# buaacyw/GaussianEditor

Measured on AMD Instinct MI355X. Metric: train iters/sec (fwd+bwd of one 1080p view per GPU + grad all-reduce), 1M Gaussians @1080p, higher is better.
Workload: dtype f32; 1 GPU; synth-v1 1000000 Gaussians SH3 (M=16, s0=0.01), 1920x1080, ring-v1 8 views, one view per GPU (BASELINE.json configs[3] shape; configs[1] bicycle.ply is not available offline); gaussians=1000000, width=1920, height=1080, views_per_rank=1, parallelism=dp1-views, view_pipeline=False, tile_bounds=reference, fast_exp=False, grad_exchange=direct, grad_exchange_route=local, grad_rows=every row of every gradient written every iteration, num_rendered=0, visible=0, pixel_instances=0, sort_key_bits=45

## Files before the change

gaussianeditor_amd/csrc/gsr_blend.hip:

```cpp
#include <limits.h>

#include <atomic>
#include <type_traits>

#include "gsr_kernels.h"

namespace gsr {

struct PixelWave {
  int tile, px, py;
  bool inside;
};

__device__ __forceinline__ bool setup_wave(const BlendArgs& a, uint32_t tile, uint32_t quad, PixelWave& pw) {
  const int tx = (int)(tile % (uint32_t)a.gx), ty = (int)(tile / (uint32_t)a.gx);
  const int lane = lane_id();
  pw.tile = (int)tile;
  pw.px = tx * TILE + (int)(quad & 1u) * QUAD + (lane & 7);
  pw.py = ty * TILE + (int)(quad >> 1) * QUAD + (lane >> 3);
  pw.inside = pw.px < a.W && pw.py < a.H;
  return __any(pw.inside) != 0;
}

struct ItemBox {
// ... 487 lines not shown
      q[10] = walk.cur.r1.y;
      stage(slot, walk.cur);
    }
    if ((uint32_t)lane >= n && (uint32_t)lane < n4) {
      float* q = &spair[lane >> 1][lane & 1];
      q[0] = q[2] = q[4] = q[6] = q[8] = q[10] = 0.f;
    }
    __syncthreads();
    uint32_t evaluated = n;
    for (uint32_t j = 0; j < n4; j += GROUP) {
      if (__all(Ts < 0.0f)) {
        evaluated = j;
        break;
      }
      float ae[GROUP], om[GROUP], w[GROUP];
      bool hit[GROUP];
#pragma unroll
      for (int pp = 0; pp < GROUP / 2; ++pp) {
        const float* q = &spair[(j >> 1) + pp][0];
        pair_alpha<FAST>(*reinterpret_cast<const float4*>(q), *reinterpret_cast<const float4*>(q + 4),
                         *reinterpret_cast<const float4*>(q + 8), pfx2, pfy2, ae + 2 * pp, om + 2 * pp);
      }
#pragma unroll
      for (int u = 0; u < GROUP; ++u) asm volatile("" : "+v"(ae[u]), "+v"(om[u]));
#pragma unroll
      for (int u = 0; u < GROUP; ++u) {
        const float test_T = Ts * om[u];
        const bool A = !(test_T < 0.0001f);
        hit[u] = A && ae[u] > 0.0f;
        w[u] = ae[u] * Ts;
        Ts = A ? test_T : -__builtin_fabsf(Ts);
      }
      group(j, hit, w);
    }
    chunk_end(min(n, evaluated));
  }
}

template <bool PROFILE, bool AUX, int SPLIT, bool FAST, bool CKPT>
__device__ __forceinline__ void forward_item(const BlendArgs& a, uint32_t tile, uint32_t quad, const float bg0, const float bg1,
                                             const float bg2, uint32_t& prof_visited, uint64_t* prof_cyc) {
  PixelWave pw;
  ItemBox box;
  if (!setup_item<SPLIT>(a, tile, quad, pw, box)) return;
  quad &= 3u;
  const int lane = lane_id();
  const uint2 range = a.ranges[pw.tile];
  const float pfx = (float)pw.px, pfy = (float)pw.py;
  (void)box;
  bool done = !pw.inside;
  float T = 1.0f;
  uint32_t last_contributor = 0;
  uint32_t evaluated = 0;

  constexpr int FWD_PAIR = 24;
  __shared__ __attribute__((aligned(16))) float sp[(WAVE / 2) * FWD_PAIR];
  const uint64_t lt_mask = (1ull << lane) - 1ull;
  const f32x2 pfx2 = {pfx, pfx}, pfy2 = {pfy, pfy};
  f32x2 C01 = {0.f, 0.f}, C2D = {0.f, 0.f};
  f32x2 S01 = {0.f, 0.f};
  float S2 = 0.f;
  constexpr bool ckpt = CKPT && !AUX;
  const uint32_t pidx = (uint32_t)((pw.py & (TILE - 1)) * TILE + (pw.px & (TILE - 1)));
  const uint32_t ck_base = ckpt ? a.ck_table[tile] : CK_NONE;
  uint32_t ck_next = (ckpt && ck_base != CK_NONE) ? (uint32_t)a.ck_pos.chunk[1] : 0xffffffffu, ck_k = 1u;
  auto stage = [&](uint32_t slot, float hA, float nB, float hC, float op, float x, float y, float z, float r, float g,
                   float b, float pos) {
    float* q = sp + (slot >> 1) * FWD_PAIR + (slot & 1u);
    q[0] = hA;
    q[2] = nB;
    q[4] = hC;
    q[6] = op;
    q[8] = x;
    q[10] = y;
    q[20] = pos;
    *reinterpret_cast<float4*>(sp + (slot >> 1) * FWD_PAIR + 12 + 4 * (slot & 1u)) = make_float4(r, g, b, z);
  };
  if (range.y > range.x) {
    ChunkWalker<true, AUX> walk(a, range.x, range.y - range.x);
    for (; walk.valid(); walk.advance()) {
      const uint64_t live_m = __ballot(!done);
      if (live_m == 0) break;
      if (ckpt && walk.chunk == ck_next) {
        if (ck_k < (uint32_t)a.ck_slots) {
          if (pw.inside) a.ck_pool[((size_t)ck_base * (uint32_t)a.ck_slots + ck_k) * (TILE * TILE) + pidx] = make_float4(T, S01.x, S01.y, S2);
          S01 = f32x2{0.f, 0.f};
          S2 = 0.f;
          if (lane == 0) atomicAdd(&a.ck_work[(size_t)tile * (uint32_t)a.ck_slots + ck_k], evaluated);
        }
        ck_k++;
        ck_next = ck_k < (uint32_t)a.ck_slots ? (uint32_t)a.ck_pos.chunk[ck_k] : 0xffffffffu;
      }
      uint64_t tc0 = 0;
      if (PROFILE) {
        tc0 = __builtin_amdgcn_s_memtime();
        prof_cyc[2]++;
      }
      const bool keep = chunk_cull(live_m, pfx - (float)(lane & 7), pfy - (float)(lane >> 3), (uint32_t)lane < walk.chunk_size(), walk.cur);
      const uint64_t m = __ballot(keep);
      if (PROFILE) prof_cyc[3] += __builtin_amdgcn_s_memtime() - tc0;
      if (m == 0) continue;
      const uint32_t cnt = (uint32_t)__popcll(m);
      const uint32_t cnt4 = (cnt + GROUP - 1) & ~(uint32_t)(GROUP - 1);
      __syncthreads();
      const float csum = (walk.cur.r2.x + walk.cur.r2.y) + (walk.cur.r2.z + walk.cur.r1.z);
      const bool bad_value = keep && !(csum - csum == 0.0f);
      if (keep)
        stage((uint32_t)__popcll(m & lt_mask), -0.5f * walk.cur.r0.x, -walk.cur.r0.y, -0.5f * walk.cur.r0.z, walk.cur.r0.w,
              walk.cur.r1.x, walk.cur.r1.y, walk.cur.r1.z, walk.cur.r2.x, walk.cur.r2.y, walk.cur.r2.z,
              __uint_as_float(walk.lane_pos() + 1u));
      if ((uint32_t)lane >= cnt && (uint32_t)lane < cnt4)
        stage((uint32_t)lane, 0.f, 0.f, 0.f, 0.f, 0.f, 0.f, 0.f, 0.f, 0.f, 0.f, 0.f);
      __syncthreads();
      uint64_t tc1 = 0;
      if (PROFILE) {
        tc1 = __builtin_amdgcn_s_memtime();
        prof_cyc[0] += tc1 - tc0;
      }
      if (!__any(bad_value)) {
        float Ts = done ? -T : T;
        for (uint32_t j = 0; j < cnt4; j += GROUP) {
          if (__all(Ts < 0.0f)) break;
          evaluated += GROUP;
          if (PROFILE) prof_visited += GROUP;
          float ae[GROUP], om[GROUP], posf[GROUP];
          f32x2 rg[GROUP], bz[GROUP];
#pragma unroll
          for (int pp = 0; pp < GROUP / 2; ++pp) {
            const float* q = sp + ((j >> 1) + pp) * FWD_PAIR;
            const float4 q0 = *reinterpret_cast<const float4*>(q), q1 = *reinterpret_cast<const float4*>(q + 4),
                         q2 = *reinterpret_cast<const float4*>(q + 8), c0 = *reinterpret_cast<const float4*>(q + 12),
                         c1 = *reinterpret_cast<const float4*>(q + 16);
            const float2 ps = *reinterpret_cast<const float2*>(q + 20);
            pair_alpha<FAST>(q0, q1, q2, pfx2, pfy2, ae + 2 * pp, om + 2 * pp);
            rg[2 * pp] = f32x2{c0.x, c0.y};
            bz[2 * pp] = f32x2{c0.z, c0.w};
            rg[2 * pp + 1] = f32x2{c1.x, c1.y};
            bz[2 * pp + 1] = f32x2{c1.z, c1.w};
            posf[2 * pp] = ps.x;
            posf[2 * pp + 1] = ps.y;
          }
#pragma unroll
          for (int u = 0; u < GROUP; ++u) asm volatile("" : "+v"(ae[u]), "+v"(om[u]));
#pragma unroll
          for (int u = 0; u < GROUP; ++u) {
            const float test_T = Ts * om[u];
            const bool A = !(test_T < 0.0001f);
            const float w = ae[u] * Ts;
            const float wz = A ? w : 0.0f;
            const f32x2 w2 = {wz, wz};
            C01 = __builtin_elementwise_fma(rg[u], w2, C01);
            C2D = __builtin_elementwise_fma(bz[u], w2, C2D);
            if (ckpt) {
              S01 = __builtin_elementwise_fma(rg[u], w2, S01);
              S2 = __builtin_fmaf(bz[u].x, wz, S2);
            }
            Ts = A ? test_T : -__builtin_fabsf(Ts);
            last_contributor = (wz > 0.0f) ? __float_as_uint(posf[u]) : last_contributor;
          }
        }
        done = Ts < 0.0f;
        T = __builtin_fabsf(Ts);
      } else {
        for (uint32_t j = 0; j < cnt4; j += GROUP) {
          if (__all(done)) break;
          evaluated += GROUP;
          if (PROFILE) prof_visited += GROUP;
          float al[GROUP], om[GROUP], posf[GROUP];
          bool ok[GROUP];
          f32x2 rg[GROUP], bz[GROUP];
  #pragma unroll
          for (int pp = 0; pp < GROUP / 2; ++pp) {
            const float* q = sp + ((j >> 1) + pp) * FWD_PAIR;
            const float4 q0 = *reinterpret_cast<const float4*>(q), q1 = *reinterpret_cast<const float4*>(q + 4),
                         q2 = *reinterpret_cast<const float4*>(q + 8), c0 = *reinterpret_cast<const float4*>(q + 12),
                         c1 = *reinterpret_cast<const float4*>(q + 16);
            const float2 ps = *reinterpret_cast<const float2*>(q + 20);
            const f32x2 hA = {q0.x, q0.y}, nB = {q0.z, q0.w}, hC = {q1.x, q1.y}, op = {q1.z, q1.w};
            const f32x2 dx = f32x2{q2.x, q2.y} - pfx2, dy = f32x2{q2.z, q2.w} - pfy2;
            const f32x2 a_ = (hA * dx) * dx;
            const f32x2 s_ = __builtin_elementwise_fma(hC * dy, dy, a_);
            const f32x2 power = __builtin_elementwise_fma(nB * dx, dy, s_);
            const f32x2 e = blend_exp2<FAST>(power);
            const f32x2 ao = op * e;
            const f32x2 a2 = {fminf(0.99f, ao.x), fminf(0.99f, ao.y)};
            const f32x2 o2 = f32x2{1.0f, 1.0f} - a2;
            al[2 * pp] = a2.x;
            al[2 * pp + 1] = a2.y;
            om[2 * pp] = o2.x;
            om[2 * pp + 1] = o2.y;
            ok[2 * pp] = !(power.x > 0.0f) && !(a2.x < 1.0f / 255.0f);
            ok[2 * pp + 1] = !(power.y > 0.0f) && !(a2.y < 1.0f / 255.0f);
            rg[2 * pp] = f32x2{c0.x, c0.y};
            bz[2 * pp] = f32x2{c0.z, c0.w};
            rg[2 * pp + 1] = f32x2{c1.x, c1.y};
            bz[2 * pp + 1] = f32x2{c1.z, c1.w};
            posf[2 * pp] = ps.x;
            posf[2 * pp + 1] = ps.y;
          }
  #pragma unroll
          for (int u = 0; u < GROUP; ++u) asm volatile("" : "+v"(al[u]), "+v"(om[u]));
  #pragma unroll
          for (int u = 0; u < GROUP; ++u) {
            const bool hit = ok[u] && !done;
            const float test_T = T * om[u];
            const bool term = hit && (test_T < 0.0001f);
            done = done || term;
            if (hit && !term) {
              const float w = al[u] * T;
              const f32x2 w2 = {w, w};
              C01 = __builtin_elementwise_fma(rg[u], w2, C01);
              C2D = __builtin_elementwise_fma(bz[u], w2, C2D);
              if (ckpt) {
                S01 = __builtin_elementwise_fma(rg[u], w2, S01);
                S2 = __builtin_fmaf(bz[u].x, w, S2);
              }
              T = test_T;
              last_contributor = __float_as_uint(posf[u]);
            }
          }
        }
      }
      if (PROFILE) prof_cyc[1] += __builtin_amdgcn_s_memtime() - tc1;
    }
  }
  const float C0 = C01.x, C1 = C01.y, C2 = C2D.x, D = C2D.y;
  const uint32_t deep = (a.work_est != nullptr || ckpt) ? wave_max_u32_dpp(last_contributor) : 0u;
  if (ckpt) {
    if (deep > a.ck_pos.pos(1u) && lane == 0) atomicMax(&a.tile_maxc[tile], deep);
    if (ck_k > 1u && pw.inside)
      a.ck_pool[((size_t)ck_base * (uint32_t)a.ck_slots + (ck_k < (uint32_t)a.ck_slots ? ck_k : 0u)) * (TILE * TILE) + pidx] = make_float4(T, S01.x, S01.y, S2);
  }
  if (a.work_est != nullptr && lane == 0) {
    if (SPLIT == 1) {
      a.work_est[4u * tile + quad] = evaluated;
      a.work_maxc[4u * tile + quad] = deep;
    } else {
      atomicMax(&a.work_est[4u * tile + quad], evaluated);
      atomicMax(&a.work_maxc[4u * tile + quad], deep);
    }
  }
  if (pw.inside) {
    const size_t pix = (size_t)pw.py * a.W + pw.px, HW = (size_t)a.H * a.W;
    if (a.final_T != nullptr) {
      a.final_T[pix] = T;
      a.n_contrib[pix] = last_contributor;
    }
    a.out_color[pix] = __builtin_fmaf(T, bg0, C0);
    a.out_color[HW + pix] = __builtin_fmaf(T, bg1, C1);
    a.out_color[2 * HW + pix] = __builtin_fmaf(T, bg2, C2);
    if (a.out_depth != nullptr) a.out_depth[pix] = D;
  }
}

template <bool PROFILE, bool AUX, int SPLIT, bool FAST, bool CKPT>
__global__ void __launch_bounds__(WAVE) __attribute__((amdgpu_waves_per_eu(4, 4))) blend_forward_kernel(const BlendArgs a) {
  uint64_t t_start = 0;
  uint32_t prof_visited = 0, prof_items = 0;
  uint64_t prof_cyc[4] = {0, 0, 0, 0};
  if (PROFILE) t_start = __builtin_amdgcn_s_memtime();
  const float bg0 = wave_uniform(a.bg[0]), bg1 = wave_uniform(a.bg[1]), bg2 = wave_uniform(a.bg[2]);
  run_work_queue<SPLIT>(a, true, [&](uint32_t tile, uint32_t quad, bool empty) __attribute__((always_inline)) {
    if (PROFILE) prof_items++;
    if (!empty) {
      forward_item<PROFILE, AUX, SPLIT, FAST, CKPT>(a, tile, quad, bg0, bg1, bg2, prof_visited, prof_cyc);
    } else {
      for_each_pixel_of_tile(a, tile, [&](size_t pix, size_t HW) __attribute__((always_inline)) {
        if (a.final_T != nullptr) {
          a.final_T[pix] = 1.0f;
          a.n_contrib[pix] = 0u;
        }
        a.out_color[pix] = __builtin_fmaf(1.0f, bg0, 0.f);
        a.out_color[HW + pix] = __builtin_fmaf(1.0f, bg1, 0.f);
        a.out_color[2 * HW + pix] = __builtin_fmaf(1.0f, bg2, 0.f);
        if (a.out_depth != nullptr) a.out_depth[pix] = 0.f;
      });
    }
  });
  if (PROFILE) {
    const uint64_t t_end = __builtin_amdgcn_s_memtime();
    if (lane_id() == 0) {
      uint64_t* rec = a.profile + (size_t)blockIdx.x * 8;
      rec[4] = prof_cyc[0];
      rec[5] = prof_cyc[1];
      rec[6] = prof_cyc[2];
      rec[7] = prof_cyc[3];
      rec[0] = t_start;
      rec[1] = t_end;
      rec[2] = ((uint64_t)xcc_id() << 32) | (uint64_t)__builtin_amdgcn_s_getreg((32 - 1) << 11 | 0 << 6 | 4);
      rec[3] = ((uint64_t)prof_items << 32) | (uint64_t)prof_visited;
    }
  }
}

__device__ __forceinline__ void wave_lds_sync() {
  __builtin_amdgcn_fence(__ATOMIC_ACQ_REL, "wavefront");
  __builtin_amdgcn_wave_barrier();
}

constexpr int BWD_WAVES = 4;
constexpr int ACC_LDS_ROW = 9;
template <bool DEPTH, bool ABS = false> constexpr int bwd_moments() { return (DEPTH ? 10 : 9) + (ABS ? 2 : 0); }
template <bool DEPTH, bool ABS = false> constexpr int bwd_lds_row() { return ABS ? (DEPTH ? 13 : 11) : DEPTH ? 11 : ACC_LDS_ROW; }
constexpr uint32_t BWD_ITEM_HALF = 0x80000000u;
constexpr uint32_t BWD_ITEM_PART = 0x40000000u;
constexpr uint32_t BWD_ITEM_SEG = 0x10000000u;
static_assert(BWD_ITEM_SEG == BWD_ITEM_SEG_BIT, "gsr_kernels.h states the bit gsr_debug_blend_backward_items counts");
constexpr int BWD_SEG_SHIFT = 20, BWD_NSEG_SHIFT = 24;
static_assert(CK_MAX <= 16, "a stride index must fit the item code's 4 bits");
constexpr uint32_t BWD_ITEM_TILE = 0x000fffffu;
static_assert(BWD_ITEM_TILE + 1u == (uint32_t)GSR_MAX_TILES, "include/gsr.h states the backward's tile limit");

__device__ __forceinline__ uint4 load_backward_item(const BlendArgs& a, uint32_t index) {
  const uint32_t code = scalar_load(a.bwd_order, index);
  const uint32_t ctile = code & BWD_ITEM_TILE;
  const uint2 crange = scalar_load(a.ranges, ctile);
  const uint4 cmax = scalar_load(reinterpret_cast<const uint4*>(a.work_maxc), ctile);
  const uint32_t r01 = max(cmax.x, cmax.y), r23 = max(cmax.z, cmax.w);
  return make_uint4(code, crange.x, (code & BWD_ITEM_HALF) ? ((code & BWD_ITEM_PART) ? r23 : r01) : max(r01, r23), crange.y - crange.x);
}
__device__ __forceinline__ float rcp_refined(float x) {
  const float r0 = __builtin_amdgcn_rcpf(x);
  return __builtin_fmaf(r0, __builtin_fmaf(-x, r0, 1.0f), r0);
}
struct RecStep {
  float T, B_acc, dL_dalpha;
};
__device__ __forceinline__ RecStep accum_rec_step(float T, float B_acc, float last_alpha, float last_cdot, float inv_one_m, float cdot) {
#pragma clang fp contract(fast)
  RecStep r;
  r.T = T * inv_one_m;
  r.B_acc = B_acc + last_alpha * (last_cdot - B_acc);
  r.dL_dalpha = (cdot - r.B_acc) * r.T;
  return r;
}
template <int NM>
__device__ __forceinline__ void geometry_moments(float (&v)[NM][GROUP], int u, float q, float dx, float dy) {
#pragma clang fp contract(fast)
  const float qx = q * dx, qy = q * dy;
  v[0][u] = q;
  v[1][u] = qx;
  v[2][u] = qy;
  v[3][u] = qx * dx;
  v[4][u] = qx * dy;
  v[5][u] = qy * dy;
}

template <bool FAST, bool SEG, bool DEPTH, bool ABS, bool ALPHA>
__device__ __forceinline__ uint32_t backward_tile(const BlendArgs& a, const uint4 item, const float bg0, const float bg1,
                                              const float bg2, float4 (*s0)[WAVE], float4 (*s1)[WAVE], float4 (*s2)[WAVE],
                                              uint32_t (*sid)[WAVE], float4 (*sco)[WAVE],
                                              float (*sacc)[WAVE][bwd_lds_row<DEPTH, ABS>()]) {
  static_assert(!(DEPTH && SEG), "depth backwards walk whole lists: the checkpoints hold no depth");
  constexpr int NM = bwd_moments<DEPTH, ABS>();
  constexpr int IABS = bwd_moments<DEPTH>();
  const int w = (int)(threadIdx.x >> 6), lane = lane_id();
  constexpr PackLanes tail = pack_lanes<NM>();
  auto tail_bit = [lane](uint64_t plane) __attribute__((always_inline)) { return (uint32_t)(plane >> (uint32_t)lane) & 1u; };
  const uint32_t tail_term = tail_bit(tail.term_bit[0]) | tail_bit(tail.term_bit[1]) << 1 | tail_bit(tail.term_bit[2]) << 2 |
                             tail_bit(tail.term_bit[3]) << 3;
  const uint32_t tail_entry = tail_bit(tail.entry_bit[0]) | tail_bit(tail.entry_bit[1]) << 1;
  const bool tail_adds = tail_bit(tail.adds) != 0u;
  uint32_t tile = item.x;
  const bool half_item = (tile & BWD_ITEM_HALF) != 0u;
  const uint32_t part = (tile & BWD_ITEM_PART) ? 1u : 0u;
  const bool seg_item = SEG && (tile & BWD_ITEM_SEG) != 0u;
  const uint32_t seg_first = (tile >> BWD_SEG_SHIFT) & 15u, seg = (tile >> BWD_NSEG_SHIFT) & 15u;
  tile &= BWD_ITEM_TILE;
  const uint32_t list_base = item.y, tile_max = item.z;
  if (tile_max == 0) return 0u;
  const uint32_t seg_lo = seg_item ? a.ck_pos.pos(seg_first) : 0u;
  const uint32_t nslots = (uint32_t)a.ck_slots;
  const uint32_t seg_hi = (seg_item && seg != nslots - 1u) ? min(tile_max, a.ck_pos.pos(seg + 1u)) : tile_max;
  if (seg_lo >= seg_hi) return 0u;
  PixelWave pw;
  const bool has_pixels = setup_wave(a, tile, half_item ? 2u * part + (uint32_t)(w >> 1) : (uint32_t)w, pw);
  const float pfx = (float)pw.px, pfy = (float)pw.py;
  const float qx0 = (float)(pw.px - (lane & 7)), qy0 = (float)(pw.py - (lane >> 3));
  if (half_item) pw.inside = pw.inside && ((lane >> 5) == (w & 1));
  const size_t HW = (size_t)a.H * a.W;
  const bool live = has_pixels && pw.inside;
  const size_t pix = live ? (size_t)pw.py * a.W + pw.px : (size_t)0;
  const float T_final_ld = a.final_T[pix];
  const uint32_t n_contrib_ld = a.n_contrib[pix];
  const float dpx_ld[3] = {a.dL_dpix[pix], a.dL_dpix[HW + pix], a.dL_dpix[2 * HW + pix]};
  const float dpd_ld = DEPTH ? a.dL_ddepth[pix] : 0.f;
  const float dpa_ld = ALPHA ? a.dL_dalpha[pix] : 0.f;
  ChunkWalker<false> walk(a, list_base + seg_lo, seg_hi - seg_lo);

  const float T_final = live ? T_final_ld : 0.f;
  float T = T_final;
  const uint32_t last_contributor = live ? n_contrib_ld : 0u;
  const uint32_t maxc = wave_max_u32_dpp(last_contributor);
  const float dpx[3] = {live ? dpx_ld[0] : 0.f, live ? dpx_ld[1] : 0.f, live ? dpx_ld[2] : 0.f};
  const float dpd = live ? dpd_ld : 0.f;
  const float dpa = live ? dpa_ld : 0.f;
  const float bg_dot_dpixel = ALPHA ? ((0.f + bg0 * dpx[0]) + bg1 * dpx[1] + bg2 * dpx[2]) - dpa
                                    : (0.f + bg0 * dpx[0]) + bg1 * dpx[1] + bg2 * dpx[2];
  const float neg_Tfinal_bg = -T_final * bg_dot_dpixel;
  const float ddelx_dx = 0.5f * a.W, ddely_dy = 0.5f * a.H;

  float B_acc = 0.f, last_cdot = 0.f;
  float last_alpha = 0.f;
  const uint64_t lt_mask = (1ull << lane) - 1ull;
  if (seg_item && last_contributor > seg_hi) {
    const uint32_t pidx = (uint32_t)((pw.py & (TILE - 1)) * TILE + (pw.px & (TILE - 1)));
    const size_t slot0 = (size_t)a.ck_table[tile] * nslots;
    uint32_t m = 0u;
#pragma unroll
    for (uint32_t k = 1u; k < (uint32_t)CK_MAX; ++k) m += (k < nslots && last_contributor - 1u >= a.ck_pos.pos(k)) ? 1u : 0u;
    float b0 = 0.f, b1 = 0.f, b2 = 0.f;
    auto add_slot = [&](uint32_t k, uint32_t top) __attribute__((always_inline)) {
      if (k > seg && k <= m) {
        const float4 sk = a.ck_pool[(slot0 + (k + 1u < top ? k + 1u : 0u)) * (TILE * TILE) + pidx];
        b0 += sk.y;
        b1 += sk.z;
        b2 += sk.w;
      }
    };
    auto sum_behind = [&](auto slots_c) __attribute__((always_inline)) {
      constexpr uint32_t S = decltype(slots_c)::value;
#pragma unroll
      for (uint32_t i = 1u; i < S; ++i) add_slot(S - i, S);
    };
    if (nslots == (uint32_t)CK_MAX / 2u) sum_behind(std::integral_constant<uint32_t, (uint32_t)CK_MAX / 2u>{});
    else if (nslots == (uint32_t)CK_MAX) sum_behind(std::integral_constant<uint32_t, (uint32_t)CK_MAX>{});
    else
      for (uint32_t k = nslots - 1u; k > seg; --k) add_slot(k, nslots);
    T = a.ck_pool[(slot0 + seg + 1u) * (TILE * TILE) + pidx].x;
    B_acc = (b0 * dpx[0] + b1 * dpx[1] + b2 * dpx[2]) / T;
  }

  auto flush = [&](uint32_t fb, uint32_t fsize) __attribute__((always_inline)) {
    const uint32_t col = (uint32_t)lane & 15u, sub = (uint32_t)lane >> 4;
    const uint32_t ia = col == ACC_MEAN2D || col == ACC_MEAN2D + 1u ? 1u
                        : col == ACC_OPACITY ? 0u
                        : col == ACC_CONIC ? 3u : col == ACC_CONIC + 1u ? 4u : col == ACC_CONIC + 3u ? 5u
                        : col >= ACC_COLOR && col < ACC_COLOR + 3u ? 6u + (col - ACC_COLOR)
                        : DEPTH && col == ACC_DEPTH ? 9u
                        : ABS && (col == ACC_ABS2D || col == ACC_ABS2D + 1u) ? (uint32_t)IABS + (col - ACC_ABS2D)
                        : (uint32_t)NM;
#pragma unroll
    for (uint32_t jj = 0; jj < 4u; ++jj) {
      const uint32_t p = 16u * (uint32_t)w + 4u * jj + sub;
      if (16u * (uint32_t)w + 4u * jj >= fsize) break;
      float* const row = sacc[fb][p];
      const bool used = p < fsize && ia < (uint32_t)NM;
      const float ma = used ? row[ia] : 0.f;
      const float mb = used && ia == 1u ? row[2] : 0.f;
      const float4 co = sco[fb][p];
      float val;
      bool nz;
      if (ia == 1u) {
        const bool xcol = col == ACC_MEAN2D;
        const float scale = xcol ? ddelx_dx : ddely_dy, c1 = xcol ? co.x : co.y, c2 = xcol ? co.y : co.z;
        val = -(scale * co.w) * (c1 * ma + c2 * mb);
        nz = ma != 0.f || mb != 0.f;
      } else if (ABS && ia >= (uint32_t)IABS) {
        val = ((col == ACC_ABS2D ? ddelx_dx : ddely_dy) * __builtin_fabsf(co.w)) * ma;
        nz = ma != 0.f;
      } else {
        const bool conic = ia >= 3u && ia <= 5u;
        val = conic ? (-0.5f * co.w) * ma : ma;
        nz = ma != 0.f;
      }
      if (used && nz) unsafeAtomicAdd(&a.acc[(size_t)sid[fb][p] * ACC_ROW + col], val);
      if (a.touched != nullptr) {
        const uint64_t nzm = __ballot(used && nz);
        if (col == 15u && p < fsize && ((nzm >> (16u * sub)) & 0xffffull) != 0ull) a.touched[sid[fb][p]] = 1;
      }
      if (p < fsize && col < (uint32_t)NM) row[col] = 0.f;
    }
  };

  uint32_t pend_size = 0u;
  for (; walk.valid(); walk.advance()) {
    const uint32_t csize = walk.chunk_size();
    const uint32_t cb = walk.chunk & 1u;
    if (w == 0 && (uint32_t)lane < csize) {
      sid[cb][lane] = walk.cur.id;
      sco[cb][lane] = walk.cur.r0;
    }
    const uint32_t pos = seg_lo + walk.lane_pos();
    const uint32_t chunk_lo = seg_hi - min(seg_hi - seg_lo, (walk.chunk + 1u) * (uint32_t)WAVE);
    const uint64_t live_m = __ballot(last_contributor > chunk_lo);
    bool keep = false;
    if (live_m != 0) keep = chunk_cull(live_m, qx0, qy0, ((uint32_t)lane < csize) && (pos < maxc), walk.cur);
    const uint64_t m = __ballot(keep);
    const uint32_t cnt = (uint32_t)__popcll(m);
    const uint32_t cnt4 = (cnt + GROUP - 1) & ~(uint32_t)(GROUP - 1);
    if (keep) {
      const uint32_t slot = (uint32_t)__popcll(m & lt_mask);
      s0[w][slot] = make_float4(-0.5f * walk.cur.r0.x, -walk.cur.r0.y, -0.5f * walk.cur.r0.z, walk.cur.r0.w);
      s1[w][slot] = make_float4(walk.cur.r1.x, walk.cur.r1.y, walk.cur.r1.z, __uint_as_float(pos));
      s2[w][slot] = make_float4(walk.cur.r2.x, walk.cur.r2.y, walk.cur.r2.z, __uint_as_float((uint32_t)lane));
    }
    if ((uint32_t)lane >= cnt && (uint32_t)lane < cnt4) {
      s0[w][lane] = make_float4(0.f, 0.f, 0.f, 0.f);
      s1[w][lane] = make_float4(0.f, 0.f, 0.f, __uint_as_float(0xffffffffu));
      s2[w][lane] = make_float4(0.f, 0.f, 0.f, __uint_as_float(0u));
    }
    wave_lds_sync();
    if (pend_size != 0u) flush(cb ^ 1u, pend_size);
    pend_size = csize;

    for (uint32_t j = 0; j < cnt4; j += GROUP) {
      float G[GROUP], al[GROUP], dxs[GROUP], dys[GROUP];
      bool contrib[GROUP];
      float4 cos_[GROUP], cols[GROUP];
      float dep[GROUP];
      bool any = false;
#pragma unroll
      for (int u = 0; u < GROUP; ++u) {
        const float4 g = s1[w][j + u];
        dep[u] = DEPTH ? g.z : 0.f;
        cos_[u] = s0[w][j + u];
        cols[u] = s2[w][j + u];
        const uint32_t c = __float_as_uint(g.w);
        dxs[u] = g.x - pfx;
        dys[u] = g.y - pfy;
        const float power = blend_power_prescaled(cos_[u].x, cos_[u].y, cos_[u].z, dxs[u], dys[u]);
        G[u] = blend_exp<FAST>(power);
        al[u] = fminf(0.99f, cos_[u].w * G[u]);
        contrib[u] = (c < last_contributor) && !(power > 0.0f) && !(al[u] < 1.0f / 255.0f);
        any = any || contrib[u];
      }
      if (!__any(any)) continue;

      float v[NM][GROUP];
      {
#pragma clang fp contract(fast)
#pragma unroll
        for (int u = 0; u < GROUP; ++u) {
          const bool on = contrib[u];
          const float alpha = on ? al[u] : 0.f;
          const float inv_one_m = rcp_refined(1.f - alpha);
          const float cdot = DEPTH ? cols[u].x * dpx[0] + cols[u].y * dpx[1] + cols[u].z * dpx[2] + dep[u] * dpd
                                   : cols[u].x * dpx[0] + cols[u].y * dpx[1] + cols[u].z * dpx[2];
          const RecStep rs = accum_rec_step(T, B_acc, last_alpha, last_cdot, inv_one_m, cdot);
          T = rs.T;
          B_acc = rs.B_acc;
          const float dL_dalpha = rs.dL_dalpha + neg_Tfinal_bg * inv_one_m;
          last_alpha = alpha;
          last_cdot = on ? cdot : last_cdot;
          const float q = on ? G[u] * dL_dalpha : 0.f;
          const float mD = alpha * T;
          geometry_moments(v, u, q, dxs[u], dys[u]);
          v[6][u] = mD * dpx[0];
          v[7][u] = mD * dpx[1];
          v[8][u] = mD * dpx[2];
          if constexpr (DEPTH) v[9][u] = mD * dpd;
          if constexpr (ABS) {
            const float qx = v[1][u], qy = v[2][u];
            v[IABS][u] = __builtin_fabsf(2.f * cos_[u].x * qx + cos_[u].y * qy);
            v[IABS + 1][u] = __builtin_fabsf(cos_[u].y * qx + 2.f * cos_[u].z * qy);
          }
        }
      }
      float tot = wave_sum4_pack<NM, !ABS>(v);
      asm volatile("" : "+v"(tot));
      if (tail_adds) {
        const uint32_t my_slot = __float_as_uint(s2[w][j + tail_entry].w);
        atomicAdd(&sacc[cb][my_slot][tail_term], tot);
      }
    }
    __syncthreads();
  }
  asm volatile("" ::"v"(walk.nxt.r0.x), "v"(walk.nxt.r1.x), "v"(walk.nxt.r2.x), "v"(walk.id_next), "v"(walk.id_next2));
  if (pend_size != 0u) flush((walk.chunk - 1u) & 1u, pend_size);
  return seg_hi - seg_lo;
}

template <bool FAST, bool SEG, bool DEPTH, bool ABS, bool ALPHA>
__global__ void __launch_bounds__(WAVE* BWD_WAVES) __attribute__((amdgpu_waves_per_eu(4, 4)))
blend_backward_kernel(const BlendArgs a) {
  constexpr int LDS_ROW = bwd_lds_row<DEPTH, ABS>();
  __shared__ float4 s0[BWD_WAVES][WAVE], s1[BWD_WAVES][WAVE], s2[BWD_WAVES][WAVE];
  __shared__ uint32_t sid[2][WAVE];
  __shared__ float4 sco[2][WAVE];
  __shared__ float sacc[2][WAVE][LDS_ROW];
  __shared__ uint32_t s_item;
  for (int i = threadIdx.x; i < 2 * WAVE * LDS_ROW; i += WAVE * BWD_WAVES) (&sacc[0][0][0])[i] = 0.f;
  __syncthreads();
  const float bg0 = wave_uniform(a.bg[0]), bg1 = wave_uniform(a.bg[1]), bg2 = wave_uniform(a.bg[2]);
  const uint32_t x = xcc_id() & 7u;
  const uint32_t nwork = a.bwd_meta[0];
  const uint32_t n_x = nwork > x ? (nwork - x + 7u) / 8u : 0u;
  uint32_t* head = a.queue + x * QUEUE_STRIDE;
  const bool prof = a.profile != nullptr;
  uint64_t t_begin = 0, t_tile = 0, longest = 0, first = 0;
  uint32_t ntiles = 0, west = 0;
  if (prof) t_begin = __builtin_amdgcn_s_memtime();
  auto run_tile = [&](uint32_t index) {
    if (prof) t_tile = __builtin_amdgcn_s_memtime();
    const uint4 item = load_backward_item(a, index);
    const uint32_t tile = item.x;
    const uint32_t tmax = backward_tile<FAST, SEG, DEPTH, ABS, ALPHA>(a, item, bg0, bg1, bg2, s0, s1, s2, sid, sco, sacc);
    if (prof) {
      const uint64_t d = __builtin_amdgcn_s_memtime() - t_tile;
      if (a.profile_items != nullptr && threadIdx.x == 0 && a.work_est != nullptr) {
        const uint32_t tt = tile & BWD_ITEM_TILE;
        uint64_t* r = a.profile_items + ((size_t)tt * 2 + ((tile & BWD_ITEM_PART) ? 1 : 0)) * 4;
        const uint4 e = reinterpret_cast<const uint4*>(a.work_est)[tt];
        r[0] = d;
        r[1] = ((uint64_t)e.x) | ((uint64_t)e.y << 16) | ((uint64_t)e.z << 32) | ((uint64_t)e.w << 48);
        r[2] = tmax;
        r[3] = tile;
      }
      if (ntiles == 0) first = d;
      longest = d > longest ? d : longest;
      ntiles++;
      if (a.work_est != nullptr) {
        const uint32_t tt = tile & BWD_ITEM_TILE;
        if (tile & BWD_ITEM_HALF) {
          const uint32_t q0 = (tile & BWD_ITEM_PART) ? 2u : 0u;
          west += a.work_est[4u * tt + q0] + a.work_est[4u * tt + q0 + 1];
        } else {
          west += a.work_est[4u * tt] + a.work_est[4u * tt + 1] + a.work_est[4u * tt + 2] + a.work_est[4u * tt + 3];
        }
      }
    }
  };
  uint32_t x0, base;
  const uint32_t q0 = first_item_of_block((uint32_t)a.units, x0, base);
  {
    const uint32_t n0 = nwork > x0 ? (nwork - x0 + 7u) / 8u : 0u;
    if (q0 < n0) run_tile(x0 + 8u * q0);
  }
  for (;;) {
    __syncthreads();
    if (threadIdx.x == 0) s_item = base + __hip_atomic_fetch_add(head, 1u, __ATOMIC_RELAXED, __HIP_MEMORY_SCOPE_AGENT);
    __syncthreads();
    const uint32_t q = s_item;
    if (q >= n_x) break;
    run_tile(x + 8u * q);
  }
  if (prof && threadIdx.x == 0) {
    uint64_t* rec = a.profile + (size_t)blockIdx.x * 8;
    rec[0] = t_begin;
    rec[1] = __builtin_amdgcn_s_memtime();
    rec[2] = ((uint64_t)xcc_id() << 32) | (uint64_t)__builtin_amdgcn_s_getreg((32 - 1) << 11 | 0 << 6 | 4);
    rec[3] = ((uint64_t)ntiles << 32) | (uint64_t)west;
    rec[4] = longest;
    rec[5] = first;
  }
  if (a.self_reset && threadIdx.x == 0) retire_queue(a.queue);
}

template <int C, int SPLIT, bool FAST>
__device__ __forceinline__ void trace_item(const BlendArgs& a, uint32_t tile, uint32_t quad) {
  PixelWave pw;
  ItemBox box;
  if (!setup_item<SPLIT>(a, tile, quad, pw, box)) return;
  const int lane = lane_id();
  const uint2 range = a.ranges[pw.tile];
  if (range.y <= range.x) return;
  (void)box;
  const size_t pix = (size_t)pw.py * a.W + pw.px, HW = (size_t)a.H * a.W;
  float Cw[C];
#pragma unroll
  for (int ch = 0; ch < C; ++ch) Cw[ch] = pw.inside ? a.image_weights[(size_t)ch * HW + pix] : 0.f;
  __shared__ uint32_t sid[WAVE];
  __shared__ float sacc[C][WAVE];
  __shared__ float scnt[WAVE];
  const bool row_end = (lane & 15) == 15;
  walk_front_to_back<FAST>(
      a, pw, range, [&](uint32_t slot, const Entry& e) __attribute__((always_inline)) { sid[slot] = e.id; },
      [&](uint32_t j, const bool(&hit)[GROUP], const float(&)[GROUP]) __attribute__((always_inline)) {
        const uint32_t e = j + ((uint32_t)lane >> 4);
#pragma unroll
        for (int ch = 0; ch < C; ++ch) {
          const float z = wave_sum4_to_rows(hit[0] ? Cw[ch] : 0.f, hit[1] ? Cw[ch] : 0.f, hit[2] ? Cw[ch] : 0.f, hit[3] ? Cw[ch] : 0.f);
          if (row_end) sacc[ch][e] = z;
        }
        const float zc = wave_sum4_to_rows(hit[0] ? 1.0f : 0.0f, hit[1] ? 1.0f : 0.0f, hit[2] ? 1.0f : 0.0f, hit[3] ? 1.0f : 0.0f);
        if (row_end) scnt[e] = zc;
      },
      [&](uint32_t evaluated) __attribute__((always_inline)) {
        __syncthreads();
        if ((uint32_t)lane < evaluated) {
          const int cn = (int)scnt[lane] * C;
          if (cn != 0) {
            const size_t id = sid[lane];
#pragma unroll
            for (int ch = 0; ch < C; ++ch) unsafeAtomicAdd(&a.weights[id * C + ch], sacc[ch][lane]);
            atomicAdd(&a.cnt[id], cn);
          }
        }
      });
}
template <int C, int SPLIT, bool FAST>
__global__ void __launch_bounds__(WAVE) trace_weights_kernel(const BlendArgs a) {
  run_work_queue<SPLIT>(a, false, [&](uint32_t tile, uint32_t quad, bool) __attribute__((always_inline)) { trace_item<C, SPLIT, FAST>(a, tile, quad); });
}

constexpr int FEAT_BLOCK = 16;
struct FeatureArgs {
  const float* features;
  float* out;
  const float* dL_dimage;
  float* dL_dfeatures;
  int C;
};

template <bool FAST>
__device__ __forceinline__ void feature_forward_item(const BlendArgs& a, const FeatureArgs& f, uint32_t tile, uint32_t quad) {
  PixelWave pw;
  ItemBox box;
  if (!setup_item<1>(a, tile, quad, pw, box)) return;
  (void)box;
  const uint2 range = a.ranges[pw.tile];
  const size_t pix = (size_t)pw.py * a.W + pw.px, HW = (size_t)a.H * a.W;
  __shared__ __align__(16) float sfeat[WAVE][FEAT_BLOCK];
  const int C = f.C;
  for (int c0 = 0; c0 < C; c0 += FEAT_BLOCK) {
    const int nch = min(FEAT_BLOCK, C - c0);
    float F[FEAT_BLOCK];
#pragma unroll
    for (int k = 0; k < FEAT_BLOCK; ++k) F[k] = 0.f;
    walk_front_to_back<FAST>(
        a, pw, range,
        [&](uint32_t slot, const Entry& e) __attribute__((always_inline)) {
          const float* __restrict__ fr = f.features + (size_t)e.id * (size_t)C + c0;
#pragma unroll
          for (int k = 0; k < FEAT_BLOCK; ++k) {
            const float v = fr[min(k, nch - 1)];
            sfeat[slot][k] = k < nch ? v : 0.f;
          }
        },
        [&](uint32_t j, const bool(&hit)[GROUP], const float(&w)[GROUP]) __attribute__((always_inline)) {
#pragma unroll
          for (int u = 0; u < GROUP; ++u) {
            if (hit[u]) {
              const float4* fp = reinterpret_cast<const float4*>(&sfeat[j + u][0]);
#pragma unroll
              for (int k4 = 0; k4 < FEAT_BLOCK / 4; ++k4) {
                const float4 v = fp[k4];
                F[4 * k4] = __builtin_fmaf(v.x, w[u], F[4 * k4]);
                F[4 * k4 + 1] = __builtin_fmaf(v.y, w[u], F[4 * k4 + 1]);
                F[4 * k4 + 2] = __builtin_fmaf(v.z, w[u], F[4 * k4 + 2]);
                F[4 * k4 + 3] = __builtin_fmaf(v.w, w[u], F[4 * k4 + 3]);
              }
            }
          }
        },
        [](uint32_t) __attribute__((always_inline)) {});
    if (pw.inside) {
#pragma unroll
      for (int k = 0; k < FEAT_BLOCK; ++k)
        if (k < nch) f.out[(size_t)(c0 + k) * HW + pix] = F[k];
    }
  }
}
template <bool FAST>
__global__ void __launch_bounds__(WAVE) __attribute__((amdgpu_waves_per_eu(4, 4)))
feature_forward_kernel(const BlendArgs a, const FeatureArgs f) {
  run_work_queue<1>(a, true, [&](uint32_t tile, uint32_t quad, bool empty) __attribute__((always_inline)) {
    if (!empty) {
      feature_forward_item<FAST>(a, f, tile, quad);
    } else {
      for_each_pixel_of_tile(a, tile, [&](size_t pix, size_t HW) __attribute__((always_inline)) {
        for (int c = 0; c < f.C; ++c) f.out[(size_t)c * HW + pix] = 0.f;
      });
    }
  });
}

constexpr int FEAT_NM = 6;
constexpr int FEAT_BWD_WAVES_PER_SIMD = 3;
constexpr int FEAT_LDS_ROW = FEAT_NM + FEAT_BLOCK + 1;
constexpr int FEAT_HALF = FEAT_BLOCK / 2;
static_assert(pack_lanes<FEAT_NM>().ok && pack_lanes<FEAT_HALF>().ok, "every moment / channel of every entry reaches a lane");
template <int NK>
__device__ __forceinline__ float wave_sum4_pack_outer(const float (&m)[GROUP], const float* g) {
  const int lane = lane_id();
  constexpr int N1 = NK * GROUP / 2, N2 = (N1 + 1) / 2, N3 = (N2 + 1) / 2, N4 = (N3 + 1) / 2, N5 = (N4 + 1) / 2;
  static_assert((N5 + 1) / 2 == 1, "six halvings leave one register");
  const bool second = (lane & 8) != 0;
  const float keep0 = second ? m[1] : m[0], give0 = second ? m[0] : m[1];
  const float keep1 = second ? m[3] : m[2], give1 = second ? m[2] : m[3];
  auto other = [](float x) __attribute__((always_inline)) {
    return __builtin_bit_cast(float, __builtin_amdgcn_update_dpp(0, __builtin_bit_cast(int, x), PackStage<8>::ctrl, 0xf, 0xf, true));
  };
  float z[N1];
#pragma unroll
  for (int k = 0; k < NK; ++k) {
    z[2 * k] = keep0 * g[k] + other(give0 * g[k]);
    z[2 * k + 1] = keep1 * g[k] + other(give1 * g[k]);
  }
  pack_stage<4, N1>(z, lane);
  pack_stage<2, N2>(z, lane);
  pack_stage<1, N3>(z, lane);
  pack_stage<32, N4>(z, lane);
  pack_stage<16, N5>(z, lane);
  return z[0];
}

template <bool FAST>
__device__ __forceinline__ void feature_backward_tile(const BlendArgs& a, const FeatureArgs& f, const uint4 item,
                                                      float4 (*s0)[WAVE], float4 (*s1)[WAVE], float (*sfeat)[WAVE][FEAT_BLOCK],
                                                      uint32_t (*sid)[WAVE], float4 (*sco)[WAVE],
                                                      float (*sacc)[WAVE][FEAT_LDS_ROW]) {
  const int w = (int)(threadIdx.x >> 6), lane = lane_id();
  constexpr PackLanes tg = pack_lanes<FEAT_NM>(), tf = pack_lanes<FEAT_HALF>();
  auto bit = [lane](uint64_t plane) __attribute__((always_inline)) { return (uint32_t)(plane >> (uint32_t)lane) & 1u; };
  const uint32_t g_term = bit(tg.term_bit[0]) | bit(tg.term_bit[1]) << 1 | bit(tg.term_bit[2]) << 2 | bit(tg.term_bit[3]) << 3;
  const uint32_t g_entry = bit(tg.entry_bit[0]) | bit(tg.entry_bit[1]) << 1;
  const bool g_adds = bit(tg.adds) != 0u;
  const uint32_t f_term = bit(tf.term_bit[0]) | bit(tf.term_bit[1]) << 1 | bit(tf.term_bit[2]) << 2 | bit(tf.term_bit[3]) << 3;
  const uint32_t f_entry = bit(tf.entry_bit[0]) | bit(tf.entry_bit[1]) << 1;
  const bool f_adds = bit(tf.adds) != 0u;
  uint32_t tile = item.x;
  const bool half_item = (tile & BWD_ITEM_HALF) != 0u;
  const uint32_t part = (tile & BWD_ITEM_PART) ? 1u : 0u;
  tile &= BWD_ITEM_TILE;
  const uint32_t list_base = item.y, tile_max = item.z;
  if (tile_max == 0) return;
  PixelWave pw;
  const bool has_pixels = setup_wave(a, tile, half_item ? 2u * part + (uint32_t)(w >> 1) : (uint32_t)w, pw);
  const float pfx = (float)pw.px, pfy = (float)pw.py;
  const float qx0 = (float)(pw.px - (lane & 7)), qy0 = (float)(pw.py - (lane >> 3));
  if (half_item) pw.inside = pw.inside && ((lane >> 5) == (w & 1));
  const size_t HW = (size_t)a.H * a.W;
  const bool live = has_pixels && pw.inside;
  const size_t pix = live ? (size_t)pw.py * a.W + pw.px : (size_t)0;
  const float T_final_ld = a.final_T[pix];
  const uint32_t n_contrib_ld = a.n_contrib[pix];
  const float T_final = live ? T_final_ld : 0.f;
  const uint32_t last_contributor = live ? n_contrib_ld : 0u;
  const uint32_t maxc = wave_max_u32_dpp(last_contributor);
  const float ddelx_dx = 0.5f * a.W, ddely_dy = 0.5f * a.H;
  const uint64_t lt_mask = (1ull << lane) - 1ull;
  const int C = f.C;
  const uint32_t fe = 16u * (uint32_t)w + ((uint32_t)lane >> 2), fc = 4u * ((uint32_t)lane & 3u);

  for (int c0 = 0; c0 < C; c0 += FEAT_BLOCK) {
    if (c0 != 0) __syncthreads();
    float gF[FEAT_BLOCK];
#pragma unroll
    for (int k = 0; k < FEAT_BLOCK; ++k) {
      const float v = f.dL_dimage[(size_t)min(c0 + k, C - 1) * HW + pix];
      gF[k] = (live && c0 + k < C) ? v : 0.f;
    }
    auto fetch = [&](uint32_t id_of_lane) __attribute__((always_inline)) {
      const uint32_t id = (uint32_t)__shfl((int)id_of_lane, (int)fe);
      const float* __restrict__ fr = f.features + (size_t)id * (size_t)C;
      float4 r;
      const int cc = c0 + (int)fc;
      r.x = fr[min(cc, C - 1)];
      r.y = fr[min(cc + 1, C - 1)];
      r.z = fr[min(cc + 2, C - 1)];
      r.w = fr[min(cc + 3, C - 1)];
      r.x = cc < C ? r.x : 0.f;
      r.y = cc + 1 < C ? r.y : 0.f;
      r.z = cc + 2 < C ? r.z : 0.f;
      r.w = cc + 3 < C ? r.w : 0.f;
      return r;
    };
    ChunkWalker<false> walk(a, list_base, tile_max);
    float4 fcur = fetch(walk.cur.id);
    float T = T_final;
    float B_acc = 0.f, last_cdot = 0.f, last_alpha = 0.f;

    auto flush = [&](uint32_t fb, uint32_t fsize) __attribute__((always_inline)) {
      const uint32_t col = (uint32_t)lane & 15u, sub = (uint32_t)lane >> 4;
      const uint32_t ia = col == ACC_MEAN2D || col == ACC_MEAN2D + 1u ? 1u
                          : col == ACC_OPACITY ? 0u
                          : col == ACC_CONIC ? 3u : col == ACC_CONIC + 1u ? 4u : col == ACC_CONIC + 3u ? 5u
                          : (uint32_t)FEAT_NM;
#pragma unroll
      for (uint32_t jj = 0; jj < 4u; ++jj) {
        const uint32_t p = 16u * (uint32_t)w + 4u * jj + sub;
        if (16u * (uint32_t)w + 4u * jj >= fsize) break;
        const bool in = p < fsize;
        float* const row = sacc[fb][in ? p : 0u];
        const bool used = in && ia < (uint32_t)FEAT_NM;
        const float ma = used ? row[ia] : 0.f;
        const float mb = used && ia == 1u ? row[2] : 0.f;
        const float fv = in ? row[FEAT_NM + col] : 0.f;
        const float4 co = sco[fb][in ? p : 0u];
        const size_t id = sid[fb][in ? p : 0u];
        float val;
        bool nz;
        if (ia == 1u) {
          const bool xcol = col == ACC_MEAN2D;
          const float scale = xcol ? ddelx_dx : ddely_dy, c1 = xcol ? co.x : co.y, c2 = xcol ? co.y : co.z;
          val = -(scale * co.w) * (c1 * ma + c2 * mb);
          nz = ma != 0.f || mb != 0.f;
        } else {
          const bool conic = ia >= 3u && ia <= 5u;
          val = conic ? (-0.5f * co.w) * ma : ma;
          nz = ma != 0.f;
        }
        if (used && nz) unsafeAtomicAdd(&a.acc[id * ACC_ROW + col], val);
        if (in && fv != 0.f && c0 + (int)col < C) unsafeAtomicAdd(&f.dL_dfeatures[id * (size_t)C + (size_t)c0 + col], fv);
        if (in) {
          row[col] = 0.f;
          if (col < (uint32_t)(FEAT_NM + FEAT_BLOCK - 16)) row[16u + col] = 0.f;
        }
      }
// ... 540 lines not shown
```

Measured before the change: 1856 view-iters/s.

## Carry partial groups across chunks and flush only used accumulator rows in backward blend

In the blend backward kernel, each wave's culled Gaussians are no longer padded up to a full GROUP per chunk. The remainder of fewer than GROUP entries is carried into the next chunk's staging area, with extra LDS slots per wave to hold the carried ids and conics. The flush now builds a compacted list of accumulator rows that were actually written, using per-wave ballot masks stored in LDS, and iterates only over those rows. This avoids wasted zero-padded inner-loop iterations and flush passes over untouched rows. The cost is extra LDS, more bookkeeping and wave syncs per chunk, and higher risk of subtle indexing bugs.

```diff
diff --git a/gaussianeditor_amd/csrc/gsr_blend.hip b/gaussianeditor_amd/csrc/gsr_blend.hip
--- a/gaussianeditor_amd/csrc/gsr_blend.hip
+++ b/gaussianeditor_amd/csrc/gsr_blend.hip
@@ -813,6 +813,10 @@
 constexpr int ACC_LDS_ROW = 9;
 template <bool DEPTH, bool ABS = false> constexpr int bwd_moments() { return (DEPTH ? 10 : 9) + (ABS ? 2 : 0); }
 template <bool DEPTH, bool ABS = false> constexpr int bwd_lds_row() { return ABS ? (DEPTH ? 13 : 11) : DEPTH ? 11 : ACC_LDS_ROW; }
+constexpr int BWD_CARRY = GROUP - 1;
+constexpr int BWD_STAGE = WAVE + GROUP;
+constexpr int BWD_SLOTS = WAVE + BWD_WAVES * BWD_CARRY;
+constexpr int BWD_LIST = (BWD_SLOTS + GROUP + 3) & ~3;
 constexpr uint32_t BWD_ITEM_HALF = 0x80000000u;
 constexpr uint32_t BWD_ITEM_PART = 0x40000000u;
 constexpr uint32_t BWD_ITEM_SEG = 0x10000000u;
@@ -859,9 +863,10 @@
 
 template <bool FAST, bool SEG, bool DEPTH, bool ABS, bool ALPHA>
 __device__ __forceinline__ uint32_t backward_tile(const BlendArgs& a, const uint4 item, const float bg0, const float bg1,
-                                              const float bg2, float4 (*s0)[WAVE], float4 (*s1)[WAVE], float4 (*s2)[WAVE],
-                                              uint32_t (*sid)[WAVE], float4 (*sco)[WAVE],
-                                              float (*sacc)[WAVE][bwd_lds_row<DEPTH, ABS>()]) {
+                                              const float bg2, float4 (*s0)[BWD_STAGE], float4 (*s1)[BWD_STAGE],
+                                              float4 (*s2)[BWD_STAGE], uint32_t (*sid)[BWD_SLOTS], float4 (*sco)[BWD_SLOTS],
+                                              float (*sacc)[BWD_SLOTS][bwd_lds_row<DEPTH, ABS>()], uint32_t (*sused)[4 * BWD_WAVES],
+                                              uint32_t (*slist)[BWD_LIST]) {
   static_assert(!(DEPTH && SEG), "depth backwards walk whole lists: the checkpoints hold no depth");
   constexpr int NM = bwd_moments<DEPTH, ABS>();
   constexpr int IABS = bwd_moments<DEPTH>();
@@ -942,8 +947,23 @@
     B_acc = (b0 * dpx[0] + b1 * dpx[1] + b2 * dpx[2]) / T;
   }
 
-  auto flush = [&](uint32_t fb, uint32_t fsize) __attribute__((always_inline)) {
-    const uint32_t col = (uint32_t)lane & 15u, sub = (uint32_t)lane >> 4;
+  auto flush = [&](uint32_t fb) __attribute__((always_inline)) {
+    uint32_t fl = (uint32_t)lane;
+    asm volatile("" : "+v"(fl));
+    const uint32_t col = fl & 15u, sub = fl >> 4;
+    int uw = (int)sused[fb][col];
+    uw |= __builtin_amdgcn_update_dpp(0, uw, 0xB1, 0xf, 0xf, false);
+    uw |= __builtin_amdgcn_update_dpp(0, uw, 0x4E, 0xf, 0xf, false);
+    const uint32_t ulo = (uint32_t)__builtin_amdgcn_readlane(uw, 0), uhi = (uint32_t)__builtin_amdgcn_readlane(uw, 4);
+    const uint32_t ucar = (uint32_t)__builtin_amdgcn_readlane(uw, 8);
+    const uint32_t n_chunk = (uint32_t)__builtin_popcount(ulo) + (uint32_t)__builtin_popcount(uhi);
+    const uint32_t n_used = n_chunk + (uint32_t)__builtin_popcount(ucar);
+    if (n_used == 0u) return;
+    const uint64_t umask = (uint64_t)uhi << 32 | ulo;
+    if ((umask >> fl) & 1ull) slist[w][__builtin_amdgcn_mbcnt_hi(uhi, __builtin_amdgcn_mbcnt_lo(ulo, 0u))] = fl;
+    if (fl < (uint32_t)(BWD_WAVES * BWD_CARRY) && ((ucar >> fl) & 1u))
+      slist[w][n_chunk + __builtin_amdgcn_mbcnt_lo(ucar, 0u)] = (uint32_t)WAVE + fl;
+    wave_lds_sync();
     const uint32_t ia = col == ACC_MEAN2D || col == ACC_MEAN2D + 1u ? 1u
                         : col == ACC_OPACITY ? 0u
                         : col == ACC_CONIC ? 3u : col == ACC_CONIC + 1u ? 4u : col == ACC_CONIC + 3u ? 5u
@@ -951,43 +971,38 @@
                         : DEPTH && col == ACC_DEPTH ? 9u
                         : ABS && (col == ACC_ABS2D || col == ACC_ABS2D + 1u) ? (uint32_t)IABS + (col - ACC_ABS2D)
                         : (uint32_t)NM;
-#pragma unroll
-    for (uint32_t jj = 0; jj < 4u; ++jj) {
-      const uint32_t p = 16u * (uint32_t)w + 4u * jj + sub;
-      if (16u * (uint32_t)w + 4u * jj >= fsize) break;
+    const bool col_used = ia < (uint32_t)NM, is_mean = ia == 1u, xcol = col == ACC_MEAN2D;
+    const bool is_abs = ABS && col_used && ia >= (uint32_t)IABS, is_conic = ia >= 3u && ia <= 5u;
+    const uint32_t ia_read = col_used ? ia : 0u;
+    const float half_wh = (is_mean ? xcol : col == ACC_ABS2D) ? ddelx_dx : ddely_dy;
+    for (uint32_t r0 = 4u * (uint32_t)w; r0 < n_used; r0 += 4u * (uint32_t)BWD_WAVES) {
+      const bool have = r0 + sub < n_used;
+      const uint32_t listed = slist[w][r0 + sub];
+      const uint32_t p = have ? listed : 0u;
       float* const row = sacc[fb][p];
-      const bool used = p < fsize && ia < (uint32_t)NM;
-      const float ma = used ? row[ia] : 0.f;
-      const float mb = used && ia == 1u ? row[2] : 0.f;
+      const bool used = have && col_used;
+      const float row_a = row[ia_read], row_b = row[2];
       const float4 co = sco[fb][p];
-      float val;
-      bool nz;
-      if (ia == 1u) {
-        const bool xcol = col == ACC_MEAN2D;
-        const float scale = xcol ? ddelx_dx : ddely_dy, c1 = xcol ? co.x : co.y, c2 = xcol ? co.y : co.z;
-        val = -(scale * co.w) * (c1 * ma + c2 * mb);
-        nz = ma != 0.f || mb != 0.f;
-      } else if (ABS && ia >= (uint32_t)IABS) {
-        val = ((col == ACC_ABS2D ? ddelx_dx : ddely_dy) * __builtin_fabsf(co.w)) * ma;
-        nz = ma != 0.f;
-      } else {
-        const bool conic = ia >= 3u && ia <= 5u;
-        val = conic ? (-0.5f * co.w) * ma : ma;
-        nz = ma != 0.f;
-      }
-      if (used && nz) unsafeAtomicAdd(&a.acc[(size_t)sid[fb][p] * ACC_ROW + col], val);
+      const uint32_t gaussian = sid[fb][p];
+      const float ma = used ? row_a : 0.f, mb = used && is_mean ? row_b : 0.f;
+      const float c1 = is_mean ? (xcol ? co.x : co.y) : 1.f, c2 = is_mean ? (xcol ? co.y : co.z) : 0.f;
+      const float f = is_mean ? -(half_wh * co.w) : is_abs ? half_wh * __builtin_fabsf(co.w) : is_conic ? -0.5f * co.w : 1.f;
+      const float val = f * (c1 * ma + c2 * mb);
+      const bool nz = ma != 0.f || mb != 0.f;
+      if (used && nz) unsafeAtomicAdd(&a.acc[(size_t)gaussian * ACC_ROW + col], val);
       if (a.touched != nullptr) {
         const uint64_t nzm = __ballot(used && nz);
-        if (col == 15u && p < fsize && ((nzm >> (16u * sub)) & 0xffffull) != 0ull) a.touched[sid[fb][p]] = 1;
-      }
-      if (p < fsize && col < (uint32_t)NM) row[col] = 0.f;
+        if (col == 15u && have && ((nzm >> (16u * sub)) & 0xffffull) != 0ull) a.touched[gaussian] = 1;
+      }
+      if (have && col < (uint32_t)NM) row[col] = 0.f;
     }
   };
 
-  uint32_t pend_size = 0u;
+  uint32_t carry = 0u;
   for (; walk.valid(); walk.advance()) {
     const uint32_t csize = walk.chunk_size();
     const uint32_t cb = walk.chunk & 1u;
+    const bool last_chunk = walk.chunk * (uint32_t)WAVE + csize == walk.count;
     if (w == 0 && (uint32_t)lane < csize) {
       sid[cb][lane] = walk.cur.id;
       sco[cb][lane] = walk.cur.r0;
@@ -998,22 +1013,34 @@
     bool keep = false;
     if (live_m != 0) keep = chunk_cull(live_m, qx0, qy0, ((uint32_t)lane < csize) && (pos < maxc), walk.cur);
     const uint64_t m = __ballot(keep);
-    const uint32_t cnt = (uint32_t)__popcll(m);
-    const uint32_t cnt4 = (cnt + GROUP - 1) & ~(uint32_t)(GROUP - 1);
+    const uint32_t cnt = carry + (uint32_t)__popcll(m);
+    const uint32_t cnt4 = (cnt + (last_chunk ? (uint32_t)(GROUP - 1) : 0u)) & ~(uint32_t)(GROUP - 1);
+    const uint32_t slot = carry + (uint32_t)__popcll(m & lt_mask);
+    {
+      const uint64_t mine = __ballot(keep && slot < cnt4);
+      const uint32_t mine_carry = cnt4 != 0u ? ((1u << carry) - 1u) << (BWD_CARRY * w) : 0u;
+      if (lane < 3) sused[cb][BWD_WAVES * lane + w] = lane == 0 ? (uint32_t)mine : lane == 1 ? (uint32_t)(mine >> 32) : mine_carry;
+    }
     if (keep) {
-      const uint32_t slot = (uint32_t)__popcll(m & lt_mask);
       s0[w][slot] = make_float4(-0.5f * walk.cur.r0.x, -walk.cur.r0.y, -0.5f * walk.cur.r0.z, walk.cur.r0.w);
       s1[w][slot] = make_float4(walk.cur.r1.x, walk.cur.r1.y, walk.cur.r1.z, __uint_as_float(pos));
       s2[w][slot] = make_float4(walk.cur.r2.x, walk.cur.r2.y, walk.cur.r2.z, __uint_as_float((uint32_t)lane));
     }
-    if ((uint32_t)lane >= cnt && (uint32_t)lane < cnt4) {
-      s0[w][lane] = make_float4(0.f, 0.f, 0.f, 0.f);
-      s1[w][lane] = make_float4(0.f, 0.f, 0.f, __uint_as_float(0xffffffffu));
-      s2[w][lane] = make_float4(0.f, 0.f, 0.f, __uint_as_float(0u));
+    if (cnt + (uint32_t)lane < cnt4) {
+      const uint32_t at = cnt + (uint32_t)lane;
+      s0[w][at] = make_float4(0.f, 0.f, 0.f, 0.f);
+      s1[w][at] = make_float4(0.f, 0.f, 0.f, __uint_as_float(0xffffffffu));
+      s2[w][at] = make_float4(0.f, 0.f, 0.f, __uint_as_float(0u));
     }
     wave_lds_sync();
-    if (pend_size != 0u) flush(cb ^ 1u, pend_size);
-    pend_size = csize;
+    if (walk.chunk != 0u) flush(cb ^ 1u);
+    if ((uint32_t)lane < carry) {
+      const uint32_t from = __float_as_uint(s2[w][lane].w), to = (uint32_t)(WAVE + BWD_CARRY * w + lane);
+      sid[cb][to] = sid[cb ^ 1u][from];
+      sco[cb][to] = sco[cb ^ 1u][from];
+      s2[w][lane].w = __uint_as_float(to);
+    }
+    wave_lds_sync();
 
     for (uint32_t j = 0; j < cnt4; j += GROUP) {
       float G[GROUP], al[GROUP], dxs[GROUP], dys[GROUP];
@@ -1075,10 +1102,17 @@
         atomicAdd(&sacc[cb][my_slot][tail_term], tot);
       }
     }
+    carry = last_chunk ? 0u : cnt & (uint32_t)(GROUP - 1);
+    if ((uint32_t)lane < carry) {
+      const float4 c0 = s0[w][cnt4 + lane], c1 = s1[w][cnt4 + lane], c2 = s2[w][cnt4 + lane];
+      s0[w][lane] = c0;
+      s1[w][lane] = c1;
+      s2[w][lane] = c2;
+    }
     __syncthreads();
   }
   asm volatile("" ::"v"(walk.nxt.r0.x), "v"(walk.nxt.r1.x), "v"(walk.nxt.r2.x), "v"(walk.id_next), "v"(walk.id_next2));
-  if (pend_size != 0u) flush((walk.chunk - 1u) & 1u, pend_size);
+  flush((walk.chunk - 1u) & 1u);
   return seg_hi - seg_lo;
 }
 
@@ -1086,12 +1120,14 @@
 __global__ void __launch_bounds__(WAVE* BWD_WAVES) __attribute__((amdgpu_waves_per_eu(4, 4)))
 blend_backward_kernel(const BlendArgs a) {
   constexpr int LDS_ROW = bwd_lds_row<DEPTH, ABS>();
-  __shared__ float4 s0[BWD_WAVES][WAVE], s1[BWD_WAVES][WAVE], s2[BWD_WAVES][WAVE];
-  __shared__ uint32_t sid[2][WAVE];
-  __shared__ float4 sco[2][WAVE];
-  __shared__ float sacc[2][WAVE][LDS_ROW];
+  __shared__ float4 s0[BWD_WAVES][BWD_STAGE], s1[BWD_WAVES][BWD_STAGE], s2[BWD_WAVES][BWD_STAGE];
+  __shared__ uint32_t sid[2][BWD_SLOTS];
+  __shared__ float4 sco[2][BWD_SLOTS];
+  __shared__ float sacc[2][BWD_SLOTS][LDS_ROW];
+  __shared__ uint32_t sused[2][4 * BWD_WAVES];
+  __shared__ uint32_t slist[BWD_WAVES][BWD_LIST];
   __shared__ uint32_t s_item;
-  for (int i = threadIdx.x; i < 2 * WAVE * LDS_ROW; i += WAVE * BWD_WAVES) (&sacc[0][0][0])[i] = 0.f;
+  for (int i = threadIdx.x; i < 2 * BWD_SLOTS * LDS_ROW; i += WAVE * BWD_WAVES) (&sacc[0][0][0])[i] = 0.f;
   __syncthreads();
   const float bg0 = wave_uniform(a.bg[0]), bg1 = wave_uniform(a.bg[1]), bg2 = wave_uniform(a.bg[2]);
   const uint32_t x = xcc_id() & 7u;
@@ -1106,7 +1142,7 @@
     if (prof) t_tile = __builtin_amdgcn_s_memtime();
     const uint4 item = load_backward_item(a, index);
     const uint32_t tile = item.x;
-    const uint32_t tmax = backward_tile<FAST, SEG, DEPTH, ABS, ALPHA>(a, item, bg0, bg1, bg2, s0, s1, s2, sid, sco, sacc);
+    const uint32_t tmax = backward_tile<FAST, SEG, DEPTH, ABS, ALPHA>(a, item, bg0, bg1, bg2, s0, s1, s2, sid, sco, sacc, sused, slist);
     if (prof) {
       const uint64_t d = __builtin_amdgcn_s_memtime() - t_tile;
       if (a.profile_items != nullptr && threadIdx.x == 0 && a.work_est != nullptr) {
```

After: 1854 view-iters/s (median of 2 runs). About the same (-0.1%).
